# MarcosRodrigoT/VIMO-CLIP

Measured on AMD Instinct MI355X. Metric: CLIP frame-embeddings/sec (whole job; TFAM fused-clips/sec and mAP parity reported in DESIGN.md/tests), higher is better.
Workload: dtype bf16; 1 GPU; CLIP ViT-L/14 frame encoder, B*T=256 u8 224x224 frames per GPU per step (BASELINE.json configs[1]), random-init weights, fp32 residual stream; parallelism=frame-sharded x1, no collective

## Files before the change

### vimo_clip_amd/csrc/attention.hip

```cpp
#include "common.h"
#include "attn_route.h"

__device__ __forceinline__ float vmax3(float a, float b, float c) { return fmaxf(fmaxf(a, b), c); }

template <typename T, int KS0, int NKS, int NC>
__device__ __forceinline__ void attn_chunk(const char* k_lds, const char* v_lds, int koff0, int koff1, const int (&voff)[4],
                                           const uint4 (&qf)[2], int Nrt, int q, float c2, float& m, f32x4 (&o)[4], f32x4& osum) {
  constexpr int NTC = 2 * NKS, NT0 = 2 * KS0;
  const int N = NC > 0 ? NC : Nrt;
  f32x4 s[NTC];
#pragma unroll
  for (int t = 0; t < NTC; ++t) {
    if (NC > 0 && 16 * (NT0 + t) >= NC) {
      s[t] = (f32x4){-INFINITY, -INFINITY, -INFINITY, -INFINITY};
      continue;
    }
    s[t] = (f32x4){0.f, 0.f, 0.f, 0.f};
    s[t] = T::mfma16(*(const uint4*)(k_lds + koff0 + (NT0 + t) * 2048), qf[0], s[t]);
    s[t] = T::mfma16(*(const uint4*)(k_lds + koff1 + (NT0 + t) * 2048), qf[1], s[t]);
  }
#pragma unroll
  for (int t = 0; t < NTC; ++t)
    if (16 * (NT0 + t) + 16 > N && !(NC > 0 && 16 * (NT0 + t) >= NC)) {
#pragma unroll
      for (int j = 0; j < 4; ++j)
        if (16 * (NT0 + t) + 4 * q + j >= N) s[t][j] = -INFINITY;
    }
  float mx = vmax3(s[0][0], s[0][1], vmax3(s[0][2], s[0][3], -INFINITY));
#pragma unroll
  for (int t = 1; t < NTC; ++t) {
    if (NC > 0 && 16 * (NT0 + t) >= NC) continue;
    mx = vmax3(vmax3(mx, s[t][0], s[t][1]), s[t][2], s[t][3]);
  }
  mx = vmax3(mx, __shfl_xor(mx, 16, 64), -INFINITY);
  mx = vmax3(mx, __shfl_xor(mx, 32, 64), -INFINITY);
  const float mnew = vmax3(m, mx, -INFINITY);
  if (KS0 > 0) {
    const float alpha = __builtin_amdgcn_exp2f((m - mnew) * c2);
#pragma unroll
    for (int dt = 0; dt < 4; ++dt) o[dt] *= alpha;
    osum *= alpha;
  }
  m = mnew;
  const float mc = mnew * c2;
  uint4 pf[NKS];
#pragma unroll
  for (int ks = 0; ks < NKS; ++ks) {
    const f32x4 a = s[2 * ks], b = s[2 * ks + 1];
    pf[ks].x = pack2<T>(__builtin_amdgcn_exp2f(__builtin_fmaf(a[0], c2, -mc)), __builtin_amdgcn_exp2f(__builtin_fmaf(a[1], c2, -mc)));
    pf[ks].y = pack2<T>(__builtin_amdgcn_exp2f(__builtin_fmaf(a[2], c2, -mc)), __builtin_amdgcn_exp2f(__builtin_fmaf(a[3], c2, -mc)));
    pf[ks].z = pack2<T>(__builtin_amdgcn_exp2f(__builtin_fmaf(b[0], c2, -mc)), __builtin_amdgcn_exp2f(__builtin_fmaf(b[1], c2, -mc)));
    pf[ks].w = pack2<T>(__builtin_amdgcn_exp2f(__builtin_fmaf(b[2], c2, -mc)), __builtin_amdgcn_exp2f(__builtin_fmaf(b[3], c2, -mc)));
  }
  const uint4 ones = make_uint4(T::ONE_PAIR, T::ONE_PAIR, T::ONE_PAIR, T::ONE_PAIR);
  auto load_v = [&](int ks, s16x4 (&v0)[4], s16x4 (&v1)[4]) {
#pragma unroll
    for (int dt = 0; dt < 4; ++dt) {
      v0[dt] = __builtin_amdgcn_ds_read_tr16_b64_v4i16((VMC_LDS s16x4*)(v_lds + voff[dt] + (KS0 + ks) * 4096));
      v1[dt] = __builtin_amdgcn_ds_read_tr16_b64_v4i16((VMC_LDS s16x4*)(v_lds + voff[dt] + (KS0 + ks) * 4096 + 2048));
    }
  };
  auto mma_v = [&](int ks, const s16x4 (&v0)[4], const s16x4 (&v1)[4]) {
    osum = T::mfma16(ones, pf[ks], osum);
#pragma unroll
    for (int dt = 0; dt < 4; ++dt) {
      uint4 vf;
      const uint2 a = __builtin_bit_cast(uint2, v0[dt]), b = __builtin_bit_cast(uint2, v1[dt]);
      vf.x = a.x; vf.y = a.y; vf.z = b.x; vf.w = b.y;
      o[dt] = T::mfma16(vf, pf[ks], o[dt]);
    }
  };
  s16x4 va0[4], va1[4], vb0[4], vb1[4];
  load_v(0, va0, va1);
#pragma unroll
  for (int ks = 0; ks < NKS; ks += 2) {
    if (ks + 1 < NKS) load_v(ks + 1, vb0, vb1);
    mma_v(ks, va0, va1);
    if (ks + 1 < NKS) {
      if (ks + 2 < NKS) load_v(ks + 2, va0, va1);
      mma_v(ks + 1, vb0, vb1);
    }
  }
}

template <typename T, int NT, int NC, int NW = 4, bool REREAD = false, bool PERSIST = false>
__global__ void __launch_bounds__(64 * NW, NW / 2) attn_vit_kernel(const uint16_t* __restrict__ qp, const uint16_t* __restrict__ kp,
                                                       const uint16_t* __restrict__ vp, uint16_t* __restrict__ out,
                                                       float* __restrict__ lse, int N, int NQ, int H, size_t ldq, size_t ldkv, float scale,
                                                       int n_bh = 0, int stagger = 0) {
  extern __shared__ __attribute__((aligned(16))) char smem[];
  constexpr int NKEYS = 16 * NT;
  char* const k_lds = smem;
  char* const v_lds = smem + NKEYS * 128;

  const int tid = threadIdx.x, lane = tid & 63, wave = tid >> 6;
  const int r = lane & 15, q = lane >> 4;
  if constexpr (PERSIST) {
    if (stagger > 0 && blockIdx.x >= (gridDim.x >> 1))
      for (int i = 0; i < stagger; ++i) __builtin_amdgcn_s_sleep(127);
  }
  for (int bh = blockIdx.x; bh < (PERSIST ? n_bh : (int)blockIdx.x + 1); bh += PERSIST ? (int)gridDim.x : 1) {
  if (PERSIST && bh != (int)blockIdx.x) __syncthreads();
  const int f = bh / H, h = bh % H;
  const int D = H * 64;
  const uint16_t* qbase = qp + (size_t)f * NQ * ldq + h * 64;
  const uint16_t* kbase = kp + (size_t)f * N * ldkv + h * 64;
  const uint16_t* vbase = vp + (size_t)f * N * ldkv + h * 64;

  {
    constexpr int NTH = 64 * NW;
    constexpr int ITERS = (NKEYS * 8 + NTH - 1) / NTH;
    uint4 kreg[ITERS], vreg[ITERS];
#pragma unroll
    for (int i = 0; i < ITERS; ++i) {
      const int idx = i * NTH + tid;
      const int row = idx >> 3, c = idx & 7;
      kreg[i] = vreg[i] = make_uint4(0, 0, 0, 0);
      if (idx < NKEYS * 8 && row < N) {
        kreg[i] = *(const uint4*)(kbase + (size_t)row * ldkv + c * 8);
        vreg[i] = *(const uint4*)(vbase + (size_t)row * ldkv + c * 8);
      }
    }
#pragma unroll
    for (int i = 0; i < ITERS; ++i) {
      const int idx = i * NTH + tid;
      const int row = idx >> 3, c = idx & 7;
      if (idx < NKEYS * 8) {
        *(uint4*)(k_lds + lds_off_x(row, c)) = kreg[i];
        *(uint4*)(v_lds + lds_off_v(row, c)) = vreg[i];
      }
    }
  }
  __syncthreads();

  const float c2 = scale * 1.4426950408889634f;
  const int nqt = (NQ + 15) >> 4;
  const int koff0 = lds_off_x(r, q), koff1 = lds_off_x(r, 4 + q);
  int voff[4];
#pragma unroll
  for (int dt = 0; dt < 4; ++dt) voff[dt] = lds_off_v(4 * q + (r >> 2), 2 * dt + ((r & 3) >> 1)) + (r & 1) * 8;
  uint4 qnext[2];
  const int w0 = (wave + bh) & (NW - 1);
#pragma unroll
  for (int kk = 0; kk < 2; ++kk) qnext[kk] = *(const uint4*)(qbase + (size_t)min(w0 * 16 + r, NQ - 1) * ldq + (4 * kk + q) * 8);
  for (int qt = w0; qt < nqt; qt += NW) {
    if constexpr (REREAD) asm volatile("" ::: "memory");
    const int qrow = qt * 16 + r;
    uint4 qf[2] = {qnext[0], qnext[1]};
    if (qt + NW < nqt) {
#pragma unroll
      for (int kk = 0; kk < 2; ++kk) qnext[kk] = *(const uint4*)(qbase + (size_t)min(qrow + 16 * NW, NQ - 1) * ldq + (4 * kk + q) * 8);
    }

    f32x4 o[4], osum = (f32x4){0.f, 0.f, 0.f, 0.f};
#pragma unroll
    for (int dt = 0; dt < 4; ++dt) o[dt] = (f32x4){0.f, 0.f, 0.f, 0.f};
    float m = -INFINITY;
    constexpr int KS = NT / 2;
    constexpr int KA = NT >= 14 ? (KS + 1) / 2 : KS;
    attn_chunk<T, 0, KA, NC>(k_lds, v_lds, koff0, koff1, voff, qf, N, q, c2, m, o, osum);
    if constexpr (KS > KA) attn_chunk<T, KA, KS - KA, NC>(k_lds, v_lds, koff0, koff1, voff, qf, N, q, c2, m, o, osum);
    const float sum = osum[0];
    const float inv = 1.0f / sum;
    if (lse != nullptr && q == 0 && qrow < NQ) lse[((size_t)f * H + h) * NQ + qrow] = m * scale + __logf(sum);
    if (qrow < NQ) {
      uint16_t* orow = out + ((size_t)f * NQ + qrow) * D + h * 64 + 4 * q;
#pragma unroll
      for (int dt = 0; dt < 4; ++dt)
        *(uint2*)(orow + 16 * dt) = make_uint2(pack2<T>(o[dt][0] * inv, o[dt][1] * inv), pack2<T>(o[dt][2] * inv, o[dt][3] * inv));
    }
  }
  }
}

template <typename T, int I>
static int launch_vit(const AttnPlan& pl, const AttnVitProblem& p, hipStream_t s) {
  constexpr AttnVitInst c = kAttnVitInsts[I];
  auto kern = attn_vit_kernel<T, c.nt, c.nc, c.nw, c.reread, c.persist>;
  static bool lds_set = false;
  if (int rc = set_max_lds(lds_set, pl.lds, kern)) return rc;
  hipLaunchKernelGGL(kern, dim3(pl.grid[0]), dim3(pl.block), pl.lds, s, (const uint16_t*)p.q, (const uint16_t*)p.k, (const uint16_t*)p.v,
                     (uint16_t*)p.out, p.lse, p.N, p.NQ, p.H, p.ldq, p.ldkv, 0.125f, p.F * p.H, pl.stagger);
  VMC_CHECK_LAUNCH();
  return 0;
}

template <typename T>
static int vit_exec(const AttnPlan& pl, const AttnVitProblem& p, hipStream_t s) {
  static_assert(kAttnVitInstCount == 12, "one case per entry of kAttnVitInsts");
  switch (pl.vit) {
    case 0: return launch_vit<T, 0>(pl, p, s); case 1: return launch_vit<T, 1>(pl, p, s); case 2: return launch_vit<T, 2>(pl, p, s);
    case 3: return launch_vit<T, 3>(pl, p, s); case 4: return launch_vit<T, 4>(pl, p, s); case 5: return launch_vit<T, 5>(pl, p, s);
    case 6: return launch_vit<T, 6>(pl, p, s); case 7: return launch_vit<T, 7>(pl, p, s); case 8: return launch_vit<T, 8>(pl, p, s);
    case 9: return launch_vit<T, 9>(pl, p, s); case 10: return launch_vit<T, 10>(pl, p, s); case 11: return launch_vit<T, 11>(pl, p, s);
  }
  return VMC_E_ARG;
}

static const AttnOverrides& attn_overrides() {
  static const AttnOverrides o = attn_overrides_from_env();
  return o;
}

static int vit_impl(const AttnVitProblem& p, void* stream) {
  const AttnPlan pl = attn_vit_route(p, attn_overrides());
  if (pl.rc) return pl.rc;
  const hipStream_t s = (hipStream_t)stream;
  if (pl.kernel != ATTN_VIT) return attn_vit_long_fwd(pl, p, s);
  return p.dtype16 == VMC_BF16 ? vit_exec<BF16>(pl, p, s) : vit_exec<F16>(pl, p, s);
}

extern "C" int vmc_attention_vit_fwd(const void* qkv, void* out, float* lse, int F, int N, int H, int dtype16, void* stream) {
  const size_t D = (size_t)H * 64;
  return vit_impl({qkv, (const uint16_t*)qkv + D, (const uint16_t*)qkv + 2 * D, out, lse, 3 * D, 3 * D, F, N, N, H, dtype16}, stream);
}

extern "C" int vmc_attention_vit_cls_fwd(const void* q_cls, const void* kv, void* out, int F, int N, int H, int dtype16, void* stream) {
  const size_t D = (size_t)H * 64;
  return vit_impl({q_cls, kv, (const uint16_t*)kv + D, out, nullptr, D, 2 * D, F, N, 1, H, dtype16}, stream);
}

template <typename T, int DH, int NT>
__global__ void __launch_bounds__(64) attn_small_kernel(const uint16_t* __restrict__ qp, const uint16_t* __restrict__ kp,
                                                        const uint16_t* __restrict__ vp, const uint8_t* __restrict__ mask,
                                                        uint16_t* __restrict__ op, float* __restrict__ lse, int H, int Tq, int Tk,
                                                        int ldq, int ldk, int ldv, int ldo, float scale, float drop_p,
                                                        uint64_t seed_arg) {
  const uint64_t seed = drop_p > 0.f ? resolve_seed(seed_arg) : 0;
  constexpr int NKEYS = 16 * NT, CH = DH / 8, RS = DH * 2 + 16, KK = DH / 32, DT = DH / 16;
  __shared__ __attribute__((aligned(16))) char k_lds[NKEYS * RS];
  __shared__ __attribute__((aligned(16))) char v_lds[NKEYS * RS];
  const int lane = threadIdx.x, r = lane & 15, q = lane >> 4;
  const int b = blockIdx.x / H, h = blockIdx.x % H;
  const uint16_t* kb = kp + (size_t)b * Tk * ldk + h * DH;
  const uint16_t* vb = vp + (size_t)b * Tk * ldv + h * DH;
  uint4 qnext[KK];
  {
    const uint16_t* qr0 = qp + ((size_t)b * Tq + min(r, Tq - 1)) * ldq + h * DH;
#pragma unroll
    for (int kk = 0; kk < KK; ++kk) qnext[kk] = *(const uint4*)(qr0 + (4 * kk + q) * 8);
  }
  {
    constexpr int ITERS = (NKEYS * CH + 63) / 64;
    uint4 kreg[ITERS], vreg[ITERS];
#pragma unroll
    for (int i = 0; i < ITERS; ++i) {
      const int idx = i * 64 + lane, row = idx / CH, c = idx % CH;
      kreg[i] = vreg[i] = make_uint4(0, 0, 0, 0);
      if (idx < NKEYS * CH && row < Tk) {
        kreg[i] = *(const uint4*)(kb + (size_t)row * ldk + c * 8);
        vreg[i] = *(const uint4*)(vb + (size_t)row * ldv + c * 8);
      }
    }
#pragma unroll
    for (int i = 0; i < ITERS; ++i) {
      const int idx = i * 64 + lane, row = idx / CH, c = idx % CH;
      if (idx < NKEYS * CH) {
        *(uint4*)(k_lds + row * RS + c * 16) = kreg[i];
        *(uint4*)(v_lds + row * RS + c * 16) = vreg[i];
      }
    }
  }
  bool live[NT][4];
#pragma unroll
  for (int nt = 0; nt < NT; ++nt)
#pragma unroll
    for (int j = 0; j < 4; ++j) {
      const int key = 16 * nt + 4 * q + j;
      live[nt][j] = key < Tk && (mask == nullptr || mask[(size_t)b * Tk + key] != 0);
    }
  __syncthreads();

  const float c2 = scale * 1.4426950408889634f;
  const uint4 ones = make_uint4(T::ONE_PAIR, T::ONE_PAIR, T::ONE_PAIR, T::ONE_PAIR);
  for (int qt = 0; qt * 16 < Tq; ++qt) {
    const int qrow = qt * 16 + r;
    uint4 qf[KK];
#pragma unroll
    for (int kk = 0; kk < KK; ++kk) qf[kk] = qnext[kk];
    if ((qt + 1) * 16 < Tq) {
      const uint16_t* qr = qp + ((size_t)b * Tq + min(qrow + 16, Tq - 1)) * ldq + h * DH;
#pragma unroll
      for (int kk = 0; kk < KK; ++kk) qnext[kk] = *(const uint4*)(qr + (4 * kk + q) * 8);
    }
    f32x4 s[NT];
#pragma unroll
    for (int nt = 0; nt < NT; ++nt) {
      s[nt] = (f32x4){0.f, 0.f, 0.f, 0.f};
#pragma unroll
      for (int kk = 0; kk < KK; ++kk)
        s[nt] = T::mfma16(*(const uint4*)(k_lds + (16 * nt + r) * RS + (4 * kk + q) * 16), qf[kk], s[nt]);
    }
    float m = -INFINITY;
#pragma unroll
    for (int nt = 0; nt < NT; ++nt)
#pragma unroll
      for (int j = 0; j < 4; ++j) {
        if (!live[nt][j]) s[nt][j] = -INFINITY;
        m = fmaxf(m, s[nt][j]);
      }
    m = fmaxf(m, __shfl_xor(m, 16, 64));
    m = fmaxf(m, __shfl_xor(m, 32, 64));
    const float mc = m * c2;
    f32x4 o[DT], osum = (f32x4){0.f, 0.f, 0.f, 0.f};
#pragma unroll
    for (int dt = 0; dt < DT; ++dt) o[dt] = (f32x4){0.f, 0.f, 0.f, 0.f};
#pragma unroll
    for (int ks = 0; ks < NT / 2; ++ks) {
      const f32x4 a = s[2 * ks], bb = s[2 * ks + 1];
      float pe[8];
#pragma unroll
      for (int j = 0; j < 4; ++j) {
        pe[j] = __builtin_amdgcn_exp2f(__builtin_fmaf(a[j], c2, -mc));
        pe[4 + j] = __builtin_amdgcn_exp2f(__builtin_fmaf(bb[j], c2, -mc));
      }
      uint4 pf = make_uint4(pack2<T>(pe[0], pe[1]), pack2<T>(pe[2], pe[3]), pack2<T>(pe[4], pe[5]), pack2<T>(pe[6], pe[7]));
      osum = T::mfma16(ones, pf, osum);
      if (drop_p > 0.f) {
        const size_t base = (((size_t)b * H + h) * Tq + min(qrow, Tq - 1)) * Tk + 32 * ks + 4 * q;
#pragma unroll
        for (int j = 0; j < 4; ++j) {
          pe[j] *= dropout_factor(drop_p, seed, base + j);
          pe[4 + j] *= dropout_factor(drop_p, seed, base + 16 + j);
        }
        pf = make_uint4(pack2<T>(pe[0], pe[1]), pack2<T>(pe[2], pe[3]), pack2<T>(pe[4], pe[5]), pack2<T>(pe[6], pe[7]));
      }
#pragma unroll
      for (int dt = 0; dt < DT; ++dt) {
        const char* p0 = v_lds + (32 * ks + 4 * q + (r >> 2)) * RS + (16 * dt + 4 * (r & 3)) * 2;
        const s16x4 v0 = __builtin_amdgcn_ds_read_tr16_b64_v4i16((VMC_LDS s16x4*)p0);
        const s16x4 v1 = __builtin_amdgcn_ds_read_tr16_b64_v4i16((VMC_LDS s16x4*)(p0 + 16 * RS));
        uint4 vf;
        const uint2 x0 = __builtin_bit_cast(uint2, v0), x1 = __builtin_bit_cast(uint2, v1);
        vf.x = x0.x; vf.y = x0.y; vf.z = x1.x; vf.w = x1.y;
        o[dt] = T::mfma16(vf, pf, o[dt]);
      }
    }
    const float sum = osum[0];
    const float inv = 1.0f / sum;
    if (qrow < Tq) {
      uint16_t* orow = op + ((size_t)b * Tq + qrow) * ldo + h * DH + 4 * q;
#pragma unroll
      for (int dt = 0; dt < DT; ++dt)
        *(uint2*)(orow + 16 * dt) = make_uint2(pack2<T>(o[dt][0] * inv, o[dt][1] * inv), pack2<T>(o[dt][2] * inv, o[dt][3] * inv));
      if (lse != nullptr && q == 0) lse[((size_t)b * H + h) * Tq + qrow] = m * scale + __logf(sum);
    }
  }
}

template <typename T>
__device__ inline float dot16(const uint16_t* __restrict__ a16, const float* __restrict__ bf, int dh) {
  float acc = 0.f;
  for (int d = 0; d < dh; d += 8) {
    const uint4 w = *(const uint4*)(a16 + d);
    float x0, x1;
    unpack2<T>(w.x, x0, x1); acc += x0 * bf[d] + x1 * bf[d + 1];
    unpack2<T>(w.y, x0, x1); acc += x0 * bf[d + 2] + x1 * bf[d + 3];
    unpack2<T>(w.z, x0, x1); acc += x0 * bf[d + 4] + x1 * bf[d + 5];
    unpack2<T>(w.w, x0, x1); acc += x0 * bf[d + 6] + x1 * bf[d + 7];
  }
  return acc;
}

template <typename T>
__global__ void __launch_bounds__(64) attn_generic_fwd(const uint16_t* __restrict__ qp, const uint16_t* __restrict__ kp,
                                                       const uint16_t* __restrict__ vp, const uint8_t* __restrict__ mask,
                                                       uint16_t* __restrict__ op, float* __restrict__ lse, int H, int Tq,
                                                       int Tk, int dh, int ldq, int ldk, int ldv, int ldo, float scale,
                                                       float drop_p, unsigned long long seed_arg) {
  const unsigned long long seed = drop_p > 0.f ? resolve_seed(seed_arg) : 0;
  __shared__ float qs[ATT_MAX_DH];
  __shared__ float ps[ATT_MAX_TK];
  const int lane = threadIdx.x;
  const int t = blockIdx.x % Tq, h = (blockIdx.x / Tq) % H, b = blockIdx.x / (Tq * H);
  const uint16_t* qrow = qp + ((size_t)b * Tq + t) * ldq + h * dh;
  for (int d = lane; d < dh; d += 64) qs[d] = T::to_f32(qrow[d]) * scale;
  __syncthreads();
  float m = -INFINITY;
  for (int key = lane; key < Tk; key += 64) {
    float s = -INFINITY;
    if (mask == nullptr || mask[(size_t)b * Tk + key]) s = dot16<T>(kp + ((size_t)b * Tk + key) * ldk + h * dh, qs, dh);
    ps[key] = s;
    m = fmaxf(m, s);
  }
  m = wave_max(m);
  float sum = 0.f;
  for (int key = lane; key < Tk; key += 64) {
    const float p = __expf(ps[key] - m);
    ps[key] = p * dropout_factor(drop_p, seed, (((size_t)b * H + h) * Tq + t) * Tk + key);
    sum += p;
  }
  sum = wave_sum(sum);
  __syncthreads();
  const float inv = 1.0f / sum;
  for (int d = lane; d < dh; d += 64) {
    float acc = 0.f;
    const uint16_t* vcol = vp + (size_t)b * Tk * ldv + h * dh + d;
    for (int key = 0; key < Tk; ++key) acc += ps[key] * T::to_f32(vcol[(size_t)key * ldv]);
    op[((size_t)b * Tq + t) * ldo + h * dh + d] = T::from_f32(acc * inv);
  }
  if (lse != nullptr && lane == 0) lse[((size_t)b * H + h) * Tq + t] = m + __logf(sum);
}

template <typename T>
__global__ void __launch_bounds__(64) attn_generic_bwd_q(const uint16_t* __restrict__ qp, const uint16_t* __restrict__ kp,
                                                         const uint16_t* __restrict__ vp, const uint8_t* __restrict__ mask,
                                                         const uint16_t* __restrict__ op, const uint16_t* __restrict__ dop,
                                                         const float* __restrict__ lse, uint16_t* __restrict__ dqp,
                                                         float* __restrict__ delta, int H, int Tq, int Tk, int dh, int ldq,
                                                         int ldk, int ldv, int ldo, int lddq, float scale, float drop_p,
                                                         unsigned long long seed_arg) {
  const unsigned long long seed = drop_p > 0.f ? resolve_seed(seed_arg) : 0;
  __shared__ float qs[ATT_MAX_DH];
  __shared__ float dos[ATT_MAX_DH];
  __shared__ float ds[ATT_MAX_TK];
  const int lane = threadIdx.x;
  const int t = blockIdx.x % Tq, h = (blockIdx.x / Tq) % H, b = blockIdx.x / (Tq * H);
  const size_t qi = ((size_t)b * Tq + t);
  float dl = 0.f;
  for (int d = lane; d < dh; d += 64) {
    qs[d] = T::to_f32(qp[qi * ldq + h * dh + d]) * scale;
    const float g = T::to_f32(dop[qi * ldo + h * dh + d]);
    dos[d] = g;
    dl += g * T::to_f32(op[qi * ldo + h * dh + d]);
  }
  dl = wave_sum(dl);
  __syncthreads();
  const float l = lse[((size_t)b * H + h) * Tq + t];
  if (lane == 0) delta[((size_t)b * H + h) * Tq + t] = dl;
  for (int key = lane; key < Tk; key += 64) {
    float dsv = 0.f;
    if (mask == nullptr || mask[(size_t)b * Tk + key]) {
      const size_t ki = (size_t)b * Tk + key;
      const float p = __expf(dot16<T>(kp + ki * ldk + h * dh, qs, dh) - l);
      const float dp = dot16<T>(vp + ki * ldv + h * dh, dos, dh);
      dsv = p * (dp * dropout_factor(drop_p, seed, (((size_t)b * H + h) * Tq + t) * Tk + key) - dl);
    }
    ds[key] = dsv;
  }
  __syncthreads();
  for (int d = lane; d < dh; d += 64) {
    float acc = 0.f;
    const uint16_t* kcol = kp + (size_t)b * Tk * ldk + h * dh + d;
    for (int key = 0; key < Tk; ++key) acc += ds[key] * T::to_f32(kcol[(size_t)key * ldk]);
    dqp[qi * lddq + h * dh + d] = T::from_f32(acc * scale);
  }
}

template <typename T>
__global__ void __launch_bounds__(64) attn_generic_bwd_kv(const uint16_t* __restrict__ qp, const uint16_t* __restrict__ kp,
                                                          const uint16_t* __restrict__ vp, const uint8_t* __restrict__ mask,
                                                          const uint16_t* __restrict__ dop, const float* __restrict__ lse,
                                                          const float* __restrict__ delta, uint16_t* __restrict__ dkp,
                                                          uint16_t* __restrict__ dvp, int H, int Tq, int Tk, int dh, int ldq,
                                                          int ldk, int ldv, int ldo, int lddk, int lddv, float scale,
                                                          float drop_p, unsigned long long seed_arg) {
  const unsigned long long seed = drop_p > 0.f ? resolve_seed(seed_arg) : 0;
  __shared__ float ks[ATT_MAX_DH];
  __shared__ float vs[ATT_MAX_DH];
  __shared__ float pbuf[ATT_MAX_TK];
  __shared__ float dsbuf[ATT_MAX_TK];
  const int lane = threadIdx.x;
  const int key = blockIdx.x % Tk, h = (blockIdx.x / Tk) % H, b = blockIdx.x / (Tk * H);
  const size_t ki = (size_t)b * Tk + key;
  const bool live = (mask == nullptr) || mask[ki];
  for (int d = lane; d < dh; d += 64) {
    ks[d] = T::to_f32(kp[ki * ldk + h * dh + d]);
    vs[d] = T::to_f32(vp[ki * ldv + h * dh + d]);
  }
  __syncthreads();
  for (int t = lane; t < Tq; t += 64) {
    float p = 0.f, dsv = 0.f;
    if (live) {
      const size_t qi = (size_t)b * Tq + t;
// ... 354 lines not shown
```

### vimo_clip_amd/csrc/common.h

```cpp
#pragma once
#include <hip/hip_runtime.h>
#include <stdint.h>

#include "../../include/vmc.h"
#include "tile_index.h"

typedef __bf16 bf16x8 __attribute__((ext_vector_type(8)));
typedef _Float16 f16x8 __attribute__((ext_vector_type(8)));
typedef float f32x4 __attribute__((ext_vector_type(4)));
typedef float f32x16 __attribute__((ext_vector_type(16)));
typedef short s16x4 __attribute__((ext_vector_type(4)));
typedef __bf16 bf16x2 __attribute__((ext_vector_type(2)));
typedef _Float16 f16x2 __attribute__((ext_vector_type(2)));
typedef float f32x2 __attribute__((ext_vector_type(2)));

#define VMC_LDS __attribute__((address_space(3)))
#define VMC_GLOBAL __attribute__((address_space(1)))

#define VMC_CHECK_LAUNCH()                          \
  do {                                              \
    hipError_t e_ = hipGetLastError();              \
    if (e_ != hipSuccess) return (int)e_;           \
  } while (0)

template <typename... K>
static inline int set_max_lds(bool& done, int bytes, K... kernels) {
  if (done) return 0;
  for (const void* k : {(const void*)kernels...}) {
    const hipError_t e = hipFuncSetAttribute(k, hipFuncAttributeMaxDynamicSharedMemorySize, bytes);
    if (e != hipSuccess) return (int)e;
  }
  done = true;
  return 0;
}

struct AttnPlan;
struct AttnVitProblem;
struct AttnFwdProblem;
struct AttnBwdProblem;
__attribute__((visibility("hidden"))) int attn_vit_long_fwd(const AttnPlan& plan, const AttnVitProblem& p, hipStream_t s);
__attribute__((visibility("hidden"))) int attn_long_fwd(const AttnPlan& plan, const AttnFwdProblem& p, hipStream_t s);
__attribute__((visibility("hidden"))) int attn_long_bwd(const AttnPlan& plan, const AttnBwdProblem& p, hipStream_t s);

struct BF16 {
  static constexpr int id = VMC_BF16;
  __device__ static inline float to_f32(uint16_t u) { return __uint_as_float(((uint32_t)u) << 16); }
  __device__ static inline uint16_t from_f32(float f) {
    __bf16 b = (__bf16)f;
    return __builtin_bit_cast(uint16_t, b);
  }
  __device__ static inline uint32_t pack(float lo, float hi) {
    return __builtin_bit_cast(uint32_t, __builtin_convertvector((f32x2){lo, hi}, bf16x2));
  }
  static constexpr uint32_t ONE_PAIR = 0x3F803F80u;
  __device__ static inline f32x4 mfma16(const uint4& a, const uint4& b, f32x4 c) {
    return __builtin_amdgcn_mfma_f32_16x16x32_bf16(__builtin_bit_cast(bf16x8, a), __builtin_bit_cast(bf16x8, b), c, 0, 0, 0);
  }
  __device__ static inline f32x16 mfma32(const uint4& a, const uint4& b, f32x16 c) {
    return __builtin_amdgcn_mfma_f32_32x32x16_bf16(__builtin_bit_cast(bf16x8, a), __builtin_bit_cast(bf16x8, b), c, 0, 0, 0);
  }
};
struct F16 {
  static constexpr int id = VMC_F16;
  __device__ static inline float to_f32(uint16_t u) { return (float)__builtin_bit_cast(_Float16, u); }
  __device__ static inline uint16_t from_f32(float f) {
    _Float16 h = (_Float16)f;
    return __builtin_bit_cast(uint16_t, h);
  }
  __device__ static inline uint32_t pack(float lo, float hi) {
    return __builtin_bit_cast(uint32_t, __builtin_convertvector((f32x2){lo, hi}, f16x2));
  }
  static constexpr uint32_t ONE_PAIR = 0x3C003C00u;
  __device__ static inline f32x4 mfma16(const uint4& a, const uint4& b, f32x4 c) {
    return __builtin_amdgcn_mfma_f32_16x16x32_f16(__builtin_bit_cast(f16x8, a), __builtin_bit_cast(f16x8, b), c, 0, 0, 0);
  }
  __device__ static inline f32x16 mfma32(const uint4& a, const uint4& b, f32x16 c) {
    return __builtin_amdgcn_mfma_f32_32x32x16_f16(__builtin_bit_cast(f16x8, a), __builtin_bit_cast(f16x8, b), c, 0, 0, 0);
  }
};

template <typename T>
__device__ inline uint32_t pack2(float lo, float hi) {
  return T::pack(lo, hi);
}
template <typename T>
__device__ inline void unpack2(uint32_t w, float& lo, float& hi) {
  lo = T::to_f32((uint16_t)(w & 0xFFFFu));
  hi = T::to_f32((uint16_t)(w >> 16));
}

__device__ inline float wave_sum(float v) {
#pragma unroll
  for (int o = 32; o > 0; o >>= 1) v += __shfl_xor(v, o, 64);
  return v;
}
__device__ inline float wave_max(float v) {
#pragma unroll
  for (int o = 32; o > 0; o >>= 1) v = fmaxf(v, __shfl_xor(v, o, 64));
  return v;
}

template <int ACT>
__device__ inline float apply_act(float x) {
  if (ACT == VMC_ACT_QUICKGELU) return x * __builtin_amdgcn_rcpf(1.0f + __builtin_amdgcn_exp2f(-2.4554669595930156f * x));
  if (ACT == VMC_ACT_GELU_ERF) return 0.5f * x * (1.0f + erff(x * 0.70710678118654752f));
  if (ACT == VMC_ACT_RELU) return fmaxf(x, 0.0f);
  return x;
}
__device__ inline float apply_act_rt(float x, int act) {
  switch (act) {
    case VMC_ACT_QUICKGELU: return apply_act<VMC_ACT_QUICKGELU>(x);
    case VMC_ACT_GELU_ERF: return apply_act<VMC_ACT_GELU_ERF>(x);
    case VMC_ACT_RELU: return apply_act<VMC_ACT_RELU>(x);
    default: return x;
  }
}
__device__ inline float act_grad_rt(float x, int act) {
  switch (act) {
    case VMC_ACT_QUICKGELU: {
      float s = 1.0f / (1.0f + __expf(-1.702f * x));
      return s * (1.0f + 1.702f * x * (1.0f - s));
    }
    case VMC_ACT_GELU_ERF: {
      float cdf = 0.5f * (1.0f + erff(x * 0.70710678118654752f));
      float pdf = 0.3989422804014327f * __expf(-0.5f * x * x);
      return cdf + x * pdf;
    }
    case VMC_ACT_RELU: return x > 0.0f ? 1.0f : 0.0f;
    default: return 1.0f;
  }
}

__device__ inline uint32_t hash32(uint64_t seed, uint64_t i) {
  uint64_t x = (i + 0x9E3779B97F4A7C15ull) ^ seed;
  x = (x ^ (x >> 30)) * 0xBF58476D1CE4E5B9ull;
  x = (x ^ (x >> 27)) * 0x94D049BB133111EBull;
  x ^= x >> 31;
  return (uint32_t)(x >> 32);
}
#define VMC_SEED_IS_PTR (1ull << 63)
__device__ inline uint64_t resolve_seed(uint64_t s) {
  return (s & VMC_SEED_IS_PTR) ? *(const uint64_t*)(uintptr_t)(s & ~VMC_SEED_IS_PTR) : s;
}
__device__ inline int pool_rows(const int* __restrict__ pool_len, int Tn) {
  if (pool_len == nullptr) return Tn;
  const int n = *pool_len;
  return n < 1 ? 1 : (n > Tn ? Tn : n);
}
__device__ inline float dropout_factor(float p, uint64_t seed, uint64_t i) {
  if (p <= 0.f) return 1.0f;
  return hash32(seed, i) >= (uint32_t)((double)p * 4294967296.0) ? 1.0f / (1.0f - p) : 0.0f;
}

__device__ __forceinline__ void adam_element(float& p, float g, float& m, float& v, float lr, float b1, float b2, float eps, float wd,
                                             int decoupled, float step_size, float inv_sqrt_bc2, float gscale) {
#pragma clang fp contract(off)
  float gr = g * gscale;
  if (decoupled) p *= (1.0f - lr * wd); else gr += wd * p;
  m = b1 * m + (1.0f - b1) * gr;
  v = b2 * v + (1.0f - b2) * gr * gr;
  p -= step_size * m / (sqrtf(v) * inv_sqrt_bc2 + eps);
}

static inline int grid_for(size_t n, int block, int max_blocks = 256 * 16) {
  size_t g = (n + block - 1) / block;
  if (g > (size_t)max_blocks) g = max_blocks;
  if (g < 1) g = 1;
  return (int)g;
}
```

### vimo_clip_amd/csrc/tile_index.h

```cpp
#pragma once

#if defined(__HIPCC__)
#define VMC_HD __host__ __device__ inline
#else
#define VMC_HD inline
#endif

VMC_HD int swz_x(int row) { return (row >> 1) & 7; }
VMC_HD int swz_w(int row) { return ((row >> 1) & 1) | (((row >> 4) & 3) << 1); }

VMC_HD int lds_off_x(int row, int chunk) { return row * 128 + ((chunk ^ swz_x(row)) << 4); }
VMC_HD int lds_off_w(int row, int chunk) { return row * 128 + ((chunk ^ swz_w(row)) << 4); }

VMC_HD int gemm_w_row(int r, int nt) { return 16 * (r >> 2) + 4 * nt + (r & 3); }
VMC_HD int gemm_c_col(int q, int nt, int j) { return 16 * q + 4 * nt + j; }

VMC_HD int g8_w_row(int r, int nt) { return 8 * (r >> 2) + 4 * nt + (r & 3); }
VMC_HD int swz_w8(int row) { return ((row >> 1) & 1) | (((row >> 3) & 3) << 1); }
VMC_HD int lds_off_w8(int row, int chunk) { return row * 128 + ((chunk ^ swz_w8(row)) << 4); }
VMC_HD void stage_src_w8(int idx, int& row, int& chunk) { row = idx >> 3; chunk = (idx & 7) ^ swz_w8(row); }

VMC_HD int g8_w_row32(int w) { return 16 * (w >> 4) + 8 * ((w >> 2) & 1) + 4 * ((w >> 3) & 1) + (w & 3); }
VMC_HD int g8_c_col32(int h, int i) { return 16 * (i >> 3) + 8 * h + (i & 7); }

VMC_HD void stage_src_x(int idx, int& row, int& chunk) { row = idx >> 3; chunk = (idx & 7) ^ swz_x(row); }
VMC_HD void stage_src_w(int idx, int& row, int& chunk) { row = idx >> 3; chunk = (idx & 7) ^ swz_w(row); }

VMC_HD int tn_swz(int row) { return ((row & 3) << 2) | ((row >> 2) & 3); }
VMC_HD void tn_stage_src(int idx, int& row, int& chunk) { row = idx >> 4; chunk = (idx & 15) ^ tn_swz(row); }
VMC_HD int tn256_a_off(int wm, int lane, int e) {
  const int r = lane & 15, g = lane >> 4, q = r >> 2, p = r & 3, row = 8 * g + q + 4 * e;
  return row * 256 + (((8 * wm + (p >> 1)) ^ tn_swz(row)) << 4) + (p & 1) * 8;
}
VMC_HD int tn256_b_off(int wn, int lane, int e) {
  const int r = lane & 15, g = lane >> 4, q = r >> 2, p = r & 3, row = 8 * g + q + 4 * e;
  return row * 256 + (((4 * wn + (p >> 1)) ^ tn_swz(row)) << 4) + (p & 1) * 8;
}

VMC_HD int xcd_remap(int bid, int nwg) {
  const int q = nwg >> 3, r = nwg & 7, xcd = bid & 7, loc = bid >> 3;
  const int base = (xcd < r) ? xcd * (q + 1) : r * (q + 1) + (xcd - r) * q;
  return base + loc;
}

VMC_HD int swz_v(int key) { return ((key >> 1) & 3) << 1; }
VMC_HD int lds_off_v(int key, int chunk) { return key * 128 + ((chunk ^ swz_v(key)) << 4); }
VMC_HD int attn_pv_key(int s, int q, int j) { return 32 * s + 16 * (j >> 2) + 4 * q + (j & 3); }
```

Measured before the change: 6273 frame-embeddings/s.

## Handle the odd 257th key with scalar dot products instead of a padded MFMA tile

For ViT attention where the key count is 16k+1 (257 for ViT-L/14 with CLS), the kernel now stages only the first NC-1 keys into the MFMA tile path and computes the leftover key separately. Its score comes from a bf16/f16 dot2 reduction across lanes, and its value contribution is a scalar FMA folded into the second chunk's online softmax. This removes a whole 16-key (effectively 32-key step) MFMA tile and its masking that existed only for one real key. In exchange it adds scalar work, extra shuffles, a special LDS region for the odd K/V row, and subtle numerical differences from rounding p to bf16.

Result: no change. 6277 frame-embeddings/s (median of 6 runs) (+0.1%).

```diff
diff --git a/vimo_clip_amd/csrc/attention.hip b/vimo_clip_amd/csrc/attention.hip
--- a/vimo_clip_amd/csrc/attention.hip
+++ b/vimo_clip_amd/csrc/attention.hip
@@ -3,9 +3,10 @@
 
 __device__ __forceinline__ float vmax3(float a, float b, float c) { return fmaxf(fmaxf(a, b), c); }
 
-template <typename T, int KS0, int NKS, int NC>
+template <typename T, int KS0, int NKS, int NC, bool ODD = false>
 __device__ __forceinline__ void attn_chunk(const char* k_lds, const char* v_lds, int koff0, int koff1, const int (&voff)[4],
-                                           const uint4 (&qf)[2], int Nrt, int q, float c2, float& m, f32x4 (&o)[4], f32x4& osum) {
+                                           const uint4 (&qf)[2], int Nrt, int q, float c2, float& m, f32x4 (&o)[4], f32x4& osum,
+                                           float sodd = -INFINITY, const char* vodd = nullptr) {
   constexpr int NTC = 2 * NKS, NT0 = 2 * KS0;
   const int N = NC > 0 ? NC : Nrt;
   f32x4 s[NTC];
@@ -34,7 +35,7 @@
   }
   mx = vmax3(mx, __shfl_xor(mx, 16, 64), -INFINITY);
   mx = vmax3(mx, __shfl_xor(mx, 32, 64), -INFINITY);
-  const float mnew = vmax3(m, mx, -INFINITY);
+  const float mnew = vmax3(m, mx, ODD ? sodd : -INFINITY);
   if (KS0 > 0) {
     const float alpha = __builtin_amdgcn_exp2f((m - mnew) * c2);
 #pragma unroll
@@ -81,6 +82,35 @@
       mma_v(ks + 1, vb0, vb1);
     }
   }
+  if constexpr (ODD) {
+    float p, p1;
+    unpack2<T>(pack2<T>(__builtin_amdgcn_exp2f(__builtin_fmaf(sodd, c2, -mc)), 0.f), p, p1);
+    osum += p;
+#pragma unroll
+    for (int dt = 0; dt < 4; ++dt) {
+      const uint2 vw = *(const uint2*)(vodd + (16 * dt + 4 * q) * 2);
+      float v[4];
+      unpack2<T>(vw.x, v[0], v[1]);
+      unpack2<T>(vw.y, v[2], v[3]);
+#pragma unroll
+      for (int j = 0; j < 4; ++j) o[dt][j] = __builtin_fmaf(p, v[j], o[dt][j]);
+    }
+  }
+}
+
+template <typename T>
+__device__ __forceinline__ float attn_odd_score(const char* kodd, const uint4 (&qf)[2], int q) {
+  float s = 0.f;
+#pragma unroll
+  for (int kk = 0; kk < 2; ++kk) {
+    const uint4 kw = *(const uint4*)(kodd + (4 * kk + q) * 16);
+    const uint32_t kws[4] = {kw.x, kw.y, kw.z, kw.w}, qws[4] = {qf[kk].x, qf[kk].y, qf[kk].z, qf[kk].w};
+#pragma unroll
+    for (int i = 0; i < 4; ++i) s = T::dot2(kws[i], qws[i], s);
+  }
+  s += __shfl_xor(s, 16, 64);
+  s += __shfl_xor(s, 32, 64);
+  return s;
 }
 
 template <typename T, int NT, int NC, int NW = 4, bool REREAD = false, bool PERSIST = false>
@@ -89,18 +119,24 @@
                                                        float* __restrict__ lse, int N, int NQ, int H, size_t ldq, size_t ldkv, float scale,
                                                        int n_bh = 0, int stagger = 0) {
   extern __shared__ __attribute__((aligned(16))) char smem[];
-  constexpr int NKEYS = 16 * NT;
+  constexpr bool ODD = NC % 16 == 1;
+  constexpr int NKEYS = ODD ? NC - 1 : 16 * NT;
+  constexpr int ODD_OFF = 2 * NKEYS * 128;
+  static_assert(!ODD || (ODD_OFF + 256 <= 16 * NT * 128 * 2 && NKEYS % 32 == 0 && NKEYS * 8 % (64 * NW) == 0),
+                "whole 32-key steps, unguarded staging, and the odd key's rows behind the images within the launch's LDS");
   char* const k_lds = smem;
   char* const v_lds = smem + NKEYS * 128;
 
-  const int tid = threadIdx.x, lane = tid & 63, wave = tid >> 6;
-  const int r = lane & 15, q = lane >> 4;
   if constexpr (PERSIST) {
     if (stagger > 0 && blockIdx.x >= (gridDim.x >> 1))
       for (int i = 0; i < stagger; ++i) __builtin_amdgcn_s_sleep(127);
   }
   for (int bh = blockIdx.x; bh < (PERSIST ? n_bh : (int)blockIdx.x + 1); bh += PERSIST ? (int)gridDim.x : 1) {
   if (PERSIST && bh != (int)blockIdx.x) __syncthreads();
+  int tid = threadIdx.x;
+  if constexpr (PERSIST) asm volatile("" : "+v"(tid));
+  const int lane = tid & 63, wave = tid >> 6;
+  const int r = lane & 15, q = lane >> 4;
   const int f = bh / H, h = bh % H;
   const int D = H * 64;
   const uint16_t* qbase = qp + (size_t)f * NQ * ldq + h * 64;
@@ -116,11 +152,13 @@
       const int idx = i * NTH + tid;
       const int row = idx >> 3, c = idx & 7;
       kreg[i] = vreg[i] = make_uint4(0, 0, 0, 0);
-      if (idx < NKEYS * 8 && row < N) {
+      if (idx < NKEYS * 8 && (ODD || row < N)) {
         kreg[i] = *(const uint4*)(kbase + (size_t)row * ldkv + c * 8);
         vreg[i] = *(const uint4*)(vbase + (size_t)row * ldkv + c * 8);
       }
     }
+    uint4 oddreg = make_uint4(0, 0, 0, 0);
+    if (ODD && tid < 16) oddreg = *(const uint4*)((tid < 8 ? kbase : vbase) + (size_t)(NC - 1) * ldkv + (tid & 7) * 8);
 #pragma unroll
     for (int i = 0; i < ITERS; ++i) {
       const int idx = i * NTH + tid;
@@ -130,6 +168,7 @@
         *(uint4*)(v_lds + lds_off_v(row, c)) = vreg[i];
       }
     }
+    if (ODD && tid < 16) *(uint4*)(smem + ODD_OFF + tid * 16) = oddreg;
   }
   __syncthreads();
 
@@ -156,10 +195,18 @@
 #pragma unroll
     for (int dt = 0; dt < 4; ++dt) o[dt] = (f32x4){0.f, 0.f, 0.f, 0.f};
     float m = -INFINITY;
-    constexpr int KS = NT / 2;
+    constexpr int KS = ODD ? NKEYS / 32 : NT / 2;
     constexpr int KA = NT >= 14 ? (KS + 1) / 2 : KS;
-    attn_chunk<T, 0, KA, NC>(k_lds, v_lds, koff0, koff1, voff, qf, N, q, c2, m, o, osum);
-    if constexpr (KS > KA) attn_chunk<T, KA, KS - KA, NC>(k_lds, v_lds, koff0, koff1, voff, qf, N, q, c2, m, o, osum);
+    if constexpr (ODD) {
+      static_assert(KS > KA, "two chunks");
+      const int odd_off = ODD_OFF + ((qt >> 5) << 8);
+      const float sodd = attn_odd_score<T>(smem + odd_off, qf, q);
+      attn_chunk<T, 0, KA, NKEYS>(k_lds, v_lds, koff0, koff1, voff, qf, N, q, c2, m, o, osum);
+      attn_chunk<T, KA, KS - KA, NKEYS, true>(k_lds, v_lds, koff0, koff1, voff, qf, N, q, c2, m, o, osum, sodd, smem + odd_off + 128);
+    } else {
+      attn_chunk<T, 0, KA, NC>(k_lds, v_lds, koff0, koff1, voff, qf, N, q, c2, m, o, osum);
+      if constexpr (KS > KA) attn_chunk<T, KA, KS - KA, NC>(k_lds, v_lds, koff0, koff1, voff, qf, N, q, c2, m, o, osum);
+    }
     const float sum = osum[0];
     const float inv = 1.0f / sum;
     if (lse != nullptr && q == 0 && qrow < NQ) lse[((size_t)f * H + h) * NQ + qrow] = m * scale + __logf(sum);
diff --git a/vimo_clip_amd/csrc/common.h b/vimo_clip_amd/csrc/common.h
--- a/vimo_clip_amd/csrc/common.h
+++ b/vimo_clip_amd/csrc/common.h
@@ -52,6 +52,9 @@
   __device__ static inline uint32_t pack(float lo, float hi) {
     return __builtin_bit_cast(uint32_t, __builtin_convertvector((f32x2){lo, hi}, bf16x2));
   }
+  __device__ static inline float dot2(uint32_t a, uint32_t b, float c) {
+    return __builtin_amdgcn_fdot2_f32_bf16(__builtin_bit_cast(bf16x2, a), __builtin_bit_cast(bf16x2, b), c, false);
+  }
   static constexpr uint32_t ONE_PAIR = 0x3F803F80u;
   __device__ static inline f32x4 mfma16(const uint4& a, const uint4& b, f32x4 c) {
     return __builtin_amdgcn_mfma_f32_16x16x32_bf16(__builtin_bit_cast(bf16x8, a), __builtin_bit_cast(bf16x8, b), c, 0, 0, 0);
@@ -69,6 +72,9 @@
   }
   __device__ static inline uint32_t pack(float lo, float hi) {
     return __builtin_bit_cast(uint32_t, __builtin_convertvector((f32x2){lo, hi}, f16x2));
+  }
+  __device__ static inline float dot2(uint32_t a, uint32_t b, float c) {
+    return __builtin_amdgcn_fdot2(__builtin_bit_cast(f16x2, a), __builtin_bit_cast(f16x2, b), c, false);
   }
   static constexpr uint32_t ONE_PAIR = 0x3C003C00u;
   __device__ static inline f32x4 mfma16(const uint4& a, const uint4& b, f32x4 c) {
```

## Stage attention K/V via direct global-to-LDS DMA and defer V wait past QK

Applied to the files above, without the earlier changes.

For non-persistent ViT attention launches, K and V are loaded with global_load_lds_dwordx4 straight into swizzled LDS instead of going through registers. The kernel waits only for the K loads before starting the first QK^T tile, and waits for V (plus the barrier) after the softmax probabilities are computed, so V transfer overlaps QK and exp work. Padded probability entries beyond NC are now zeroed instead of going through exp. The change relies on inline asm for m0 handling and vmcnt counting, which adds fragility in exchange for less staging latency and fewer register round-trips.

Result: no change. 6458 frame-embeddings/s before, 6485 frame-embeddings/s after (median of 3 runs) (+0.4%).

```diff
diff --git a/vimo_clip_amd/csrc/attention.hip b/vimo_clip_amd/csrc/attention.hip
--- a/vimo_clip_amd/csrc/attention.hip
+++ b/vimo_clip_amd/csrc/attention.hip
@@ -1,11 +1,14 @@
+#include <type_traits>
+
 #include "common.h"
 #include "attn_route.h"
 
 __device__ __forceinline__ float vmax3(float a, float b, float c) { return fmaxf(fmaxf(a, b), c); }
 
-template <typename T, int KS0, int NKS, int NC>
+template <typename T, int KS0, int NKS, int NC, typename VReady>
 __device__ __forceinline__ void attn_chunk(const char* k_lds, const char* v_lds, int koff0, int koff1, const int (&voff)[4],
-                                           const uint4 (&qf)[2], int Nrt, int q, float c2, float& m, f32x4 (&o)[4], f32x4& osum) {
+                                           const uint4 (&qf)[2], int Nrt, int q, float c2, float& m, f32x4 (&o)[4], f32x4& osum,
+                                           VReady&& v_ready) {
   constexpr int NTC = 2 * NKS, NT0 = 2 * KS0;
   const int N = NC > 0 ? NC : Nrt;
   f32x4 s[NTC];
@@ -47,11 +50,17 @@
 #pragma unroll
   for (int ks = 0; ks < NKS; ++ks) {
     const f32x4 a = s[2 * ks], b = s[2 * ks + 1];
-    pf[ks].x = pack2<T>(__builtin_amdgcn_exp2f(__builtin_fmaf(a[0], c2, -mc)), __builtin_amdgcn_exp2f(__builtin_fmaf(a[1], c2, -mc)));
-    pf[ks].y = pack2<T>(__builtin_amdgcn_exp2f(__builtin_fmaf(a[2], c2, -mc)), __builtin_amdgcn_exp2f(__builtin_fmaf(a[3], c2, -mc)));
-    pf[ks].z = pack2<T>(__builtin_amdgcn_exp2f(__builtin_fmaf(b[0], c2, -mc)), __builtin_amdgcn_exp2f(__builtin_fmaf(b[1], c2, -mc)));
-    pf[ks].w = pack2<T>(__builtin_amdgcn_exp2f(__builtin_fmaf(b[2], c2, -mc)), __builtin_amdgcn_exp2f(__builtin_fmaf(b[3], c2, -mc)));
-  }
+    pf[ks].x = pf[ks].y = pf[ks].z = pf[ks].w = 0u;
+    if (!(NC > 0 && 16 * (NT0 + 2 * ks) >= NC)) {
+      pf[ks].x = pack2<T>(__builtin_amdgcn_exp2f(__builtin_fmaf(a[0], c2, -mc)), __builtin_amdgcn_exp2f(__builtin_fmaf(a[1], c2, -mc)));
+      pf[ks].y = pack2<T>(__builtin_amdgcn_exp2f(__builtin_fmaf(a[2], c2, -mc)), __builtin_amdgcn_exp2f(__builtin_fmaf(a[3], c2, -mc)));
+    }
+    if (!(NC > 0 && 16 * (NT0 + 2 * ks + 1) >= NC)) {
+      pf[ks].z = pack2<T>(__builtin_amdgcn_exp2f(__builtin_fmaf(b[0], c2, -mc)), __builtin_amdgcn_exp2f(__builtin_fmaf(b[1], c2, -mc)));
+      pf[ks].w = pack2<T>(__builtin_amdgcn_exp2f(__builtin_fmaf(b[2], c2, -mc)), __builtin_amdgcn_exp2f(__builtin_fmaf(b[3], c2, -mc)));
+    }
+  }
+  v_ready(pf);
   const uint4 ones = make_uint4(T::ONE_PAIR, T::ONE_PAIR, T::ONE_PAIR, T::ONE_PAIR);
   auto load_v = [&](int ks, s16x4 (&v0)[4], s16x4 (&v1)[4]) {
 #pragma unroll
@@ -64,9 +73,7 @@
     osum = T::mfma16(ones, pf[ks], osum);
 #pragma unroll
     for (int dt = 0; dt < 4; ++dt) {
-      uint4 vf;
-      const uint2 a = __builtin_bit_cast(uint2, v0[dt]), b = __builtin_bit_cast(uint2, v1[dt]);
-      vf.x = a.x; vf.y = a.y; vf.z = b.x; vf.w = b.y;
+      const uint4 vf = __builtin_bit_cast(uint4, __builtin_shufflevector(v0[dt], v1[dt], 0, 1, 2, 3, 4, 5, 6, 7));
       o[dt] = T::mfma16(vf, pf[ks], o[dt]);
     }
   };
@@ -80,6 +87,30 @@
       if (ks + 2 < NKS) load_v(ks + 2, va0, va1);
       mma_v(ks + 1, vb0, vb1);
     }
+  }
+}
+
+__device__ __forceinline__ void attn_glds16(const uint16_t* gsrc, uint32_t lds_dst) {
+  unsigned keep;
+  asm volatile("s_mov_b32 %0, m0\n\ts_mov_b32 m0, %2\n\ts_nop 0\n\tglobal_load_lds_dwordx4 %1, off\n\ts_mov_b32 m0, %0"
+               : "=&s"(keep) : "v"(gsrc), "s"(lds_dst) : "memory");
+}
+typedef uint32_t u32x4 __attribute__((ext_vector_type(4)));
+__device__ __forceinline__ void attn_gload16(u32x4& dst, const uint16_t* gsrc) {
+  asm volatile("global_load_dwordx4 %0, %1, off" : "=v"(dst) : "v"(gsrc) : "memory");
+}
+template <int K>
+__device__ __forceinline__ void attn_pin(uint4 (&pf)[K]) {
+#pragma unroll
+  for (int i = 0; i < K; ++i) asm volatile("" : "+v"(pf[i].x), "+v"(pf[i].y), "+v"(pf[i].z), "+v"(pf[i].w));
+}
+template <int I>
+__device__ __forceinline__ void attn_wait_vm(int n) {
+  if constexpr (I == 0) {
+    asm volatile("s_waitcnt vmcnt(0)" ::: "memory");
+  } else {
+    if (n >= I) asm volatile("s_waitcnt vmcnt(%0)" ::"n"(I) : "memory");
+    else attn_wait_vm<I - 1>(n);
   }
 }
 
@@ -90,11 +121,13 @@
                                                        int n_bh = 0, int stagger = 0) {
   extern __shared__ __attribute__((aligned(16))) char smem[];
   constexpr int NKEYS = 16 * NT;
+  constexpr bool DMA = !PERSIST;
   char* const k_lds = smem;
   char* const v_lds = smem + NKEYS * 128;
 
-  const int tid = threadIdx.x, lane = tid & 63, wave = tid >> 6;
+  const int tid = threadIdx.x, lane = tid & 63, wave = __builtin_amdgcn_readfirstlane(tid >> 6);
   const int r = lane & 15, q = lane >> 4;
+  const int NK = NC > 0 ? NC : N;
   if constexpr (PERSIST) {
     if (stagger > 0 && blockIdx.x >= (gridDim.x >> 1))
       for (int i = 0; i < stagger; ++i) __builtin_amdgcn_s_sleep(127);
@@ -107,7 +140,55 @@
   const uint16_t* kbase = kp + (size_t)f * N * ldkv + h * 64;
   const uint16_t* vbase = vp + (size_t)f * N * ldkv + h * 64;
 
-  {
+  const float c2 = scale * 1.4426950408889634f;
+  const int nqt = (NQ + 15) >> 4;
+  const int w0 = (wave + bh) & (NW - 1);
+  uint4 qnext[2];
+
+  if constexpr (DMA) {
+    constexpr int NP = 2 * NT;
+    constexpr int ITERS = (NP + NW - 1) / NW;
+    const int npd = attn_stage_pieces(NK);
+    const uint32_t k_dst = (uint32_t)(uintptr_t)(VMC_LDS char*)k_lds, v_dst = (uint32_t)(uintptr_t)(VMC_LDS char*)v_lds;
+    u32x4 qa[2];
+#pragma unroll
+    for (int kk = 0; kk < 2; ++kk) attn_gload16(qa[kk], qbase + (size_t)min(w0 * 16 + r, NQ - 1) * ldq + (4 * kk + q) * 8);
+#pragma unroll
+    for (int i = 0; i < ITERS; ++i) {
+      const int p = i * NW + wave;
+      if (p < npd) {
+        int key, c;
+        attn_stage_src_k(p, lane, key, c);
+        attn_glds16(kbase + (size_t)min(key, NK - 1) * ldkv + c * 8, k_dst + p * 1024);
+      }
+    }
+#pragma unroll
+    for (int i = 0; i < ITERS; ++i) {
+      const int p = i * NW + wave;
+      if (p < npd) {
+        int key, c;
+        attn_stage_src_v(p, lane, key, c);
+        attn_glds16(vbase + (size_t)min(key, NK - 1) * ldkv + c * 8, v_dst + p * 1024);
+      }
+    }
+#pragma unroll
+    for (int i = 0; i < ITERS; ++i) {
+      const int p = i * NW + wave;
+      if (p >= npd && p < NP) {
+        *(uint4*)(k_lds + p * 1024 + lane * 16) = make_uint4(0, 0, 0, 0);
+        *(uint4*)(v_lds + p * 1024 + lane * 16) = make_uint4(0, 0, 0, 0);
+      }
+    }
+    attn_wait_vm<ITERS>(npd / NW);
+    asm volatile("" : "+v"(qa[0]), "+v"(qa[1]));
+#pragma unroll
+    for (int kk = 0; kk < 2; ++kk) qnext[kk] = make_uint4(qa[kk].x, qa[kk].y, qa[kk].z, qa[kk].w);
+    if (((npd - 1) & (NW - 1)) == wave && attn_stage_pad_lane(NK, lane))
+      *(uint4*)(k_lds + (npd - 1) * 1024 + lane * 16) = make_uint4(0, 0, 0, 0);
+    asm volatile("s_waitcnt lgkmcnt(0)" ::: "memory");
+    __builtin_amdgcn_s_barrier();
+    asm volatile("" ::: "memory");
+  } else {
     constexpr int NTH = 64 * NW;
     constexpr int ITERS = (NKEYS * 8 + NTH - 1) / NTH;
     uint4 kreg[ITERS], vreg[ITERS];
@@ -130,20 +211,29 @@
         *(uint4*)(v_lds + lds_off_v(row, c)) = vreg[i];
       }
     }
-  }
-  __syncthreads();
-
-  const float c2 = scale * 1.4426950408889634f;
-  const int nqt = (NQ + 15) >> 4;
+    __syncthreads();
+#pragma unroll
+    for (int kk = 0; kk < 2; ++kk) qnext[kk] = *(const uint4*)(qbase + (size_t)min(w0 * 16 + r, NQ - 1) * ldq + (4 * kk + q) * 8);
+  }
+  auto v_wait = [&](auto&... pf) __attribute__((always_inline)) {
+    (attn_pin(pf), ...);
+    __builtin_amdgcn_sched_barrier(0);
+    asm volatile("s_waitcnt vmcnt(0)" ::: "memory");
+    if constexpr (DMA) {
+      const int npd = attn_stage_pieces(NK);
+      if (((npd - 1) & (NW - 1)) == wave && attn_stage_pad_lane(NK, lane))
+        *(uint4*)(v_lds + (npd - 1) * 1024 + lane * 16) = make_uint4(0, 0, 0, 0);
+    }
+    asm volatile("s_waitcnt lgkmcnt(0)" ::: "memory");
+    __builtin_amdgcn_s_barrier();
+    asm volatile("" ::: "memory");
+  };
+
   const int koff0 = lds_off_x(r, q), koff1 = lds_off_x(r, 4 + q);
   int voff[4];
 #pragma unroll
   for (int dt = 0; dt < 4; ++dt) voff[dt] = lds_off_v(4 * q + (r >> 2), 2 * dt + ((r & 3) >> 1)) + (r & 1) * 8;
-  uint4 qnext[2];
-  const int w0 = (wave + bh) & (NW - 1);
-#pragma unroll
-  for (int kk = 0; kk < 2; ++kk) qnext[kk] = *(const uint4*)(qbase + (size_t)min(w0 * 16 + r, NQ - 1) * ldq + (4 * kk + q) * 8);
-  for (int qt = w0; qt < nqt; qt += NW) {
+  auto tile = [&](int qt, auto&& v_ready) __attribute__((always_inline)) {
     if constexpr (REREAD) asm volatile("" ::: "memory");
     const int qrow = qt * 16 + r;
     uint4 qf[2] = {qnext[0], qnext[1]};
@@ -158,8 +248,9 @@
     float m = -INFINITY;
     constexpr int KS = NT / 2;
     constexpr int KA = NT >= 14 ? (KS + 1) / 2 : KS;
-    attn_chunk<T, 0, KA, NC>(k_lds, v_lds, koff0, koff1, voff, qf, N, q, c2, m, o, osum);
-    if constexpr (KS > KA) attn_chunk<T, KA, KS - KA, NC>(k_lds, v_lds, koff0, koff1, voff, qf, N, q, c2, m, o, osum);
+    auto no_wait = [](auto&...) {};
+    attn_chunk<T, 0, KA, NC>(k_lds, v_lds, koff0, koff1, voff, qf, N, q, c2, m, o, osum, v_ready);
+    if constexpr (KS > KA) attn_chunk<T, KA, KS - KA, NC>(k_lds, v_lds, koff0, koff1, voff, qf, N, q, c2, m, o, osum, no_wait);
     const float sum = osum[0];
     const float inv = 1.0f / sum;
     if (lse != nullptr && q == 0 && qrow < NQ) lse[((size_t)f * H + h) * NQ + qrow] = m * scale + __logf(sum);
@@ -169,7 +260,14 @@
       for (int dt = 0; dt < 4; ++dt)
         *(uint2*)(orow + 16 * dt) = make_uint2(pack2<T>(o[dt][0] * inv, o[dt][1] * inv), pack2<T>(o[dt][2] * inv, o[dt][3] * inv));
     }
-  }
+  };
+  if constexpr (DMA) {
+    if (w0 < nqt) tile(w0, v_wait);
+    else v_wait();
+  } else if (w0 < nqt) {
+    tile(w0, [](auto&...) {});
+  }
+  for (int qt = w0 + NW; qt < nqt; qt += NW) tile(qt, [](auto&...) {});
   }
 }
 
diff --git a/vimo_clip_amd/csrc/tile_index.h b/vimo_clip_amd/csrc/tile_index.h
--- a/vimo_clip_amd/csrc/tile_index.h
+++ b/vimo_clip_amd/csrc/tile_index.h
@@ -45,4 +45,11 @@
 
 VMC_HD int swz_v(int key) { return ((key >> 1) & 3) << 1; }
 VMC_HD int lds_off_v(int key, int chunk) { return key * 128 + ((chunk ^ swz_v(key)) << 4); }
+VMC_HD void attn_stage_src_k(int piece, int lane, int& key, int& chunk) { stage_src_x(piece * 64 + lane, key, chunk); }
+VMC_HD void attn_stage_src_v(int piece, int lane, int& key, int& chunk) {
+  key = piece * 8 + (lane >> 3);
+  chunk = (lane & 7) ^ swz_v(key);
+}
+VMC_HD int attn_stage_pieces(int N) { return (N + 7) >> 3; }
+VMC_HD bool attn_stage_pad_lane(int N, int lane) { return (attn_stage_pieces(N) - 1) * 8 + (lane >> 3) >= N; }
 VMC_HD int attn_pv_key(int s, int q, int j) { return 32 * s + 16 * (j >> 2) + 4 * q + (j & 3); }
```
